# jhamrick/bayesian-quadrature

Hardware: AMD Instinct MI355X
Metric: bq_fit_posterior_throughput (higher is better)
Workload: dtype f64; 1 GPU; C2: d=1 N=1024 M=256 Gaussian integrand, w=dx, s=1e-3; curve_workload=C5 shard: 64 x (d=1 N=2048 M=256), w=dx, s=1e-2, on_curve=True, bordered_system=1344

## Files before the change

### bayesian-quadrature_amd/csrc/k_panel.hip

```cpp
#include "host.h"
#include "gram.h"
#include "trsm.h"
#include "slab.h"

namespace bqh {

template <int D>
void launch_assemble_d(bq_ctx *c, const double *pts, long pstride, const double *y, long ystride,
                       const GaussParams *gp, int gpstride, double *A, long lda, long astride,
                       Layout L, int batch, const FirstStep &fs, int jcols)
{
    dim3 grid((L.ntot + 127) / 128, ((jcols > 0 ? jcols : L.ntot) + 63) / 64, batch);
    if (!fs.S0) {
        hipLaunchKernelGGL(assemble_kernel<D>, grid, dim3(256), 0, c->cur, pts, pstride, y, ystride,
                           gp, gpstride, A, lda, astride, L);
        return;
    }
    const bool regs = c->cfg.first_regs != 0;
    if (regs && grid.y < 3)
        grid.y = 3;
    const long wgs = (long)grid.x * grid.y * grid.z;
    const bool w8 = c->cfg.potf2_8w && wgs <= 2L * c->cus;
#define BQ_ASM_FIRST(NW_, REGS_, STAMP_)                                                           \
    hipLaunchKernelGGL((assemble_first_kernel<D, NW_, REGS_, STAMP_>), grid, dim3(64 * NW_), 0,    \
                       c->cur, pts, pstride, y, ystride, gp, gpstride, A, lda, astride, L, fs.S0,  \
                       fs.lds, fs.sstride, fs.dinv, (long)BQ_DINV_STRIDE, fs.info, fs.scal,        \
                       fs.stamps)
    if constexpr (D == 1) {
        if (fs.stamps) {
            if (w8 && regs)
                BQ_ASM_FIRST(8, true, true);
            else if (w8)
                BQ_ASM_FIRST(8, false, true);
            else if (regs)
                BQ_ASM_FIRST(4, true, true);
            else
                BQ_ASM_FIRST(4, false, true);
            return;
        }
    }
    if (w8 && regs)
        BQ_ASM_FIRST(8, true, false);
    else if (w8)
        BQ_ASM_FIRST(8, false, false);
    else if (regs)
        BQ_ASM_FIRST(4, true, false);
    else
        BQ_ASM_FIRST(4, false, false);
#undef BQ_ASM_FIRST
}

int launch_assemble(bq_ctx *c, int d, const double *pts, long pstride, const double *y,
                    long ystride, const GaussParams *gp, int gpstride, double *A, long lda,
                    long astride, Layout L, int batch, const FirstStep &fs, int jcols)
{
    if (jcols < 0 || (jcols & 63) || jcols > L.ntot || (jcols > 0 && fs.S0))
        return fail(c, BQ_ERR_BAD_ARG, "assemble: column limit");
    if (fs.stamps && (!fs.S0 || d != 1))
        return fail(c, BQ_ERR_BAD_ARG, "assemble: the stamped first launch is one-dimensional");
    const double cols = jcols > 0 ? jcols : L.ntot;
    Bracket br(c, BQ_K_GRAM, 8.0 * cols * (L.ntot - 0.5 * cols + 0.5) * batch);
    switch (d) {
    case 1: launch_assemble_d<1>(c, pts, pstride, y, ystride, gp, gpstride, A, lda, astride, L, batch, fs, jcols); break;
    case 2: launch_assemble_d<2>(c, pts, pstride, y, ystride, gp, gpstride, A, lda, astride, L, batch, fs, jcols); break;
    case 3: launch_assemble_d<3>(c, pts, pstride, y, ystride, gp, gpstride, A, lda, astride, L, batch, fs, jcols); break;
    case 4: launch_assemble_d<4>(c, pts, pstride, y, ystride, gp, gpstride, A, lda, astride, L, batch, fs, jcols); break;
    case 5: launch_assemble_d<5>(c, pts, pstride, y, ystride, gp, gpstride, A, lda, astride, L, batch, fs, jcols); break;
    case 6: launch_assemble_d<6>(c, pts, pstride, y, ystride, gp, gpstride, A, lda, astride, L, batch, fs, jcols); break;
    case 7: launch_assemble_d<7>(c, pts, pstride, y, ystride, gp, gpstride, A, lda, astride, L, batch, fs, jcols); break;
    case 8: launch_assemble_d<8>(c, pts, pstride, y, ystride, gp, gpstride, A, lda, astride, L, batch, fs, jcols); break;
    default: return fail(c, BQ_ERR_BAD_ARG, "d must be in 1..%d", BQ_MAXD);
    }
    HIPCHK(c, hipGetLastError());
    return BQ_OK;
}

int launch_assemble_region(bq_ctx *c, const GramSeed &sd, double *A, long lda, long astride, int m,
                           int n, int batch)
{
    if (m <= 0 || n <= 0)
        return BQ_OK;
    if ((m & 63) || (n & 63) || (sd.r & 63) || (sd.c & 63))
        return fail(c, BQ_ERR_BAD_ARG, "assemble_region: multiples of 64");
    Bracket br(c, BQ_K_GRAM, 8.0 * m * n * batch);
    const dim3 grid((m + 127) / 128, n / 64, batch);
#define BQ_ASM_REGION(D_)                                                                          \
    case D_:                                                                                       \
        hipLaunchKernelGGL(assemble_region_kernel<D_>, grid, dim3(256), 0, c->cur, sd.pts,         \
                           sd.pstride, sd.y, sd.ystride, sd.gp, sd.gpstride, A, lda, astride, sd.L, \
                           sd.r, sd.c, m, n);                                                      \
        break;
    switch (sd.d) {
        BQ_ASM_REGION(1)
        BQ_ASM_REGION(2)
        BQ_ASM_REGION(3)
        BQ_ASM_REGION(4)
        BQ_ASM_REGION(5)
        BQ_ASM_REGION(6)
        BQ_ASM_REGION(7)
        BQ_ASM_REGION(8)
    default:
        return fail(c, BQ_ERR_BAD_ARG, "d must be in 1..%d", BQ_MAXD);
    }
#undef BQ_ASM_REGION
    HIPCHK(c, hipGetLastError());
    return BQ_OK;
}

int launch_potf2(bq_ctx *c, double *A, long lda, long astride, int j0, double *dinv, long dstride,
                 int *info, int batch)
{
    Bracket br(c, BQ_K_POTF2, 64.0 * 64 * 64 / 3.0 * batch);
    if (c->cfg.potf2_8w && batch <= c->cus)
        hipLaunchKernelGGL(potf2_kernel<8>, dim3(1, 1, batch), dim3(512), 0, c->cur, A, lda, astride,
                           j0, dinv, dstride, info);
    else
        hipLaunchKernelGGL(potf2_kernel<4>, dim3(1, 1, batch), dim3(256), 0, c->cur, A, lda, astride,
                           j0, dinv, dstride, info);
    HIPCHK(c, hipGetLastError());
    return BQ_OK;
}

int launch_potrf_wg(bq_ctx *c, double *A, long lda, long astride, int kb, double *rec, long rstride,
                    int *info, int col0, int batch)
{
    Bracket br(c, BQ_K_POTF2, (double)kb * kb * kb / 3.0 * batch);
    hipLaunchKernelGGL(potrf_wg_kernel, dim3(batch), dim3(512), 0, c->cur, A, lda, astride, kb, rec,
                       rstride, info, col0);
    HIPCHK(c, hipGetLastError());
    return BQ_OK;
}

int launch_trsm_blk(bq_ctx *c, double *X, long ldx, long xstride, int m, const double *L11,
                    long ldl, long lstride, const double *dinv, long dstride, int batch)
{
    if (m <= 0)
        return BQ_OK;
    Bracket br(c, BQ_K_TRSM, 64.0 * 64 * (double)m * batch);
    hipLaunchKernelGGL(trsm_blk_kernel, dim3((m + 63) / 64, 1, batch), dim3(256), 0, c->cur, X, ldx,
                       xstride, m, L11, ldl, lstride, dinv, dstride);
    HIPCHK(c, hipGetLastError());
    return BQ_OK;
}

int launch_diag_winv(bq_ctx *c, const double *L, long ldl, int npad, double *dw)
{
    hipLaunchKernelGGL(diag_winv_kernel, dim3(npad / 64), dim3(256), 0, c->stream, L, ldl, dw);
    HIPCHK(c, hipGetLastError());
    return BQ_OK;
}

int launch_panel_step(bq_ctx *c, double *A, long lda, long astride, int batch, int nrb,
                      double *Sin, double *Sout, long lds, long sstride, int K0, int j0,
                      double *dinv_in, double *dinv_out, int has_next, int first, double *SL,
                      int *info, double work)
{
    Bracket br(c, BQ_K_GEMM, work);
    const bool beside_bulk = c->sharing != 0 && (long)nrb * batch > 64;
    if (c->cfg.potf2_8w && !beside_bulk && (long)nrb * batch <= c->cus)
        hipLaunchKernelGGL(panel_step_kernel<8>, dim3(nrb, 1, batch), dim3(512), 0, c->cur, A, lda,
                           astride, Sin, Sout, lds, sstride, K0, j0, dinv_in, dinv_out,
                           (long)BQ_DINV_STRIDE, has_next, first, SL, info);
    else
        hipLaunchKernelGGL(panel_step_kernel<4>, dim3(nrb, 1, batch), dim3(256), 0, c->cur, A, lda,
                           astride, Sin, Sout, lds, sstride, K0, j0, dinv_in, dinv_out,
                           (long)BQ_DINV_STRIDE, has_next, first, SL, info);
    HIPCHK(c, hipGetLastError());
    return BQ_OK;
}

int launch_slab_first(bq_ctx *c, double *A, long lda, long astride, int batch, double *S, long lds,
                      long sstride, int ntot, double *dinv, int *info, int col0, long dstride)
{
    Bracket br(c, BQ_K_POTF2, 64.0 * 64 * 64 / 3.0 * batch);
    hipLaunchKernelGGL(slab_first_kernel, dim3(ntot / 64, 1, batch), dim3(256), 0, c->cur, A, lda,
                       astride, S, lds, sstride, ntot, dinv, dstride, info, col0);
    HIPCHK(c, hipGetLastError());
    return BQ_OK;
}

static long slab8_limit(const bq_ctx *c)
{
    return (long)(c->cfg.slab8_rounds > 1 ? c->cfg.slab8_rounds : 1) * c->cus;
}

int launch_slab_step(bq_ctx *c, double *A, long lda, long astride, int batch, double *Sin,
                     double *Sout, long lds, long sstride, int ntot, int j0, double *dinv_in,
                     double *dinv_out, int fnext, int last, int *info, int col0,
                     const SlabOut &out, long long *stamps, double work, long dstride)
{
    const int T = (ntot - j0 - 64) / 64;
    Bracket br(c, BQ_K_SYRK_SMALL, work);
    const long wgs = (long)T * (T + 1) / 2 * batch;
    const bool w8 = c->cfg.potf2_8w && wgs <= slab8_limit(c);
    if (stamps && w8)
        hipLaunchKernelGGL((slab_step_kernel<true, 8>), dim3(T * (T + 1) / 2, 1, batch), dim3(512), 0,
                           c->cur, A, lda, astride, Sin, Sout, lds, sstride, ntot, j0, dinv_in,
                           dinv_out, dstride, fnext, last, info, col0, stamps, out);
    else if (stamps)
        hipLaunchKernelGGL((slab_step_kernel<true, 4>), dim3(T * (T + 1) / 2, 1, batch), dim3(256), 0,
                           c->cur, A, lda, astride, Sin, Sout, lds, sstride, ntot, j0, dinv_in,
                           dinv_out, dstride, fnext, last, info, col0, stamps, out);
    else if (w8)
        hipLaunchKernelGGL((slab_step_kernel<false, 8>), dim3(T * (T + 1) / 2, 1, batch), dim3(512),
                           0, c->cur, A, lda, astride, Sin, Sout, lds, sstride, ntot, j0, dinv_in,
                           dinv_out, dstride, fnext, last, info, col0,
                           (long long *)nullptr, out);
    else
        hipLaunchKernelGGL((slab_step_kernel<false, 4>), dim3(T * (T + 1) / 2, 1, batch), dim3(256),
                           0, c->cur, A, lda, astride, Sin, Sout, lds, sstride, ntot, j0, dinv_in,
                           dinv_out, dstride, fnext, last, info, col0,
                           (long long *)nullptr, out);
    HIPCHK(c, hipGetLastError());
    return BQ_OK;
}

}
```

### bayesian-quadrature_amd/csrc/launch_config.h

```cpp
#pragma once
#include <hip/hip_runtime.h>

#pragma GCC visibility push(default)
#include "../../include/bqhip.h"
#pragma GCC visibility pop

#include <cstdio>
#include <cstdlib>

#define BQ_LAUNCH_SWITCHES(X)                                                                       \
    X(lookahead, "BQ_LOOKAHEAD", 1)                                                                 \
                 \
    X(la_min, "BQ_LA_MIN", 3072)                                                                    \
                                 \
    X(diag_first, "BQ_DIAG_FIRST", 1)                                                               \
              \
    X(df_sweep, "BQ_DF_SWEEP", 1)                                                                   \
                                               \
    X(df_wg, "BQ_DF_WG", -1)                                                                        \
                                             \
    X(df_wg_rows, "BQ_DF_WG_ROWS", 1000)                                                            \
                       \
    X(df_early, "BQ_DF_EARLY", 1)                                                                   \
                                                  \
    X(trsv_flow, "BQ_TRSV_FLOW", 1)                                                                 \
                                                                                      \
    X(pair_border, "BQ_PAIR_BORDER", 1)                                                             \
            \
    X(solve_kcopy, "BQ_SOLVE_KCOPY", 1)                                                             \
                                              \
    X(gemm_lds, "BQ_GEMM_LDS", 1)                                                                   \
                             \
    X(fold_readout, "BQ_FOLD_READOUT", 1)                                                           \
                                                                           \
    X(asm_fuse, "BQ_ASM_FUSE", 1)                                                                   \
                                                                            \
    X(potf2_8w, "BQ_POTF2_8W", 1)                                                                   \
                           \
    X(first_regs, "BQ_FIRST_REGS", 1)                                                               \
                              \
    X(slab8_rounds, "BQ_SLAB8_ROUNDS", 1 << 20)                                                     \
                        \
    X(gemm_ksplit, "BQ_GEMM_KSPLIT", 1)                                                             \
                  \
    X(gemm_tile, "BQ_GEMM_TILE", 0)                                                                 \
                                                                                     \
    X(use_graph, "BQ_GRAPH", 1)                                                                     \
               \
    X(nb_override, nullptr, 0)

struct LaunchConfig {
#define X(member, env, def) int member = def;
    BQ_LAUNCH_SWITCHES(X)
#undef X
    static LaunchConfig from_env()
    {
        LaunchConfig cfg;
        static const struct {
            const char *env;
            int LaunchConfig::*member;
        } switches[] = {
#define X(member, env, def) {env, &LaunchConfig::member},
            BQ_LAUNCH_SWITCHES(X)
#undef X
        };
        for (const auto &sw : switches)
            if (const char *e = sw.env ? std::getenv(sw.env) : nullptr)
                cfg.*sw.member = std::atoi(e);
        return cfg;
    }
    friend bool operator==(const LaunchConfig &a, const LaunchConfig &b)
    {
#define X(member, env, def) if (a.member != b.member) return false;
        BQ_LAUNCH_SWITCHES(X)
#undef X
        return true;
    }
    friend bool operator!=(const LaunchConfig &a, const LaunchConfig &b) { return !(a == b); }
};

struct CaptureStats {
    long captures = 0;
    long replays = 0;
    long drops = 0;
};

struct CapturedSeq {
    hipGraph_t graph = nullptr;
    hipGraphExec_t exec = nullptr;
    enum State { NotTried, Ready, Unavailable } state = NotTried;
    LaunchConfig cfg;
    CapturedSeq() = default;
    CapturedSeq(const CapturedSeq &) = delete;
    CapturedSeq &operator=(const CapturedSeq &) = delete;
    ~CapturedSeq() { drop(); }
    void drop()
    {
        if (exec)
            (void)hipGraphExecDestroy(exec);
        if (graph)
            (void)hipGraphDestroy(graph);
        exec = nullptr;
        graph = nullptr;
        state = NotTried;
    }
    template <class Ctx, class F>
    int run(Ctx *c, F &&enqueue)
    {
        if (!c->cfg.use_graph || c->prof || !c->own_stream || c->cur != c->stream)
            return enqueue();
        if (state == Ready && cfg != c->cfg) {
            drop();
            ++c->graphs.drops;
        }
        if (state == NotTried) {
            state = Unavailable;
            cfg = c->cfg;
            if (hipStreamBeginCapture(c->stream, hipStreamCaptureModeRelaxed) == hipSuccess) {
                const int st = enqueue();
                const hipError_t e = hipStreamEndCapture(c->stream, &graph);
                if (st == BQ_OK && e == hipSuccess && graph &&
                    hipGraphInstantiate(&exec, graph, nullptr, nullptr, 0) == hipSuccess) {
                    state = Ready;
                    ++c->graphs.captures;
                }
            }
            if (state != Ready) {
                exec = nullptr;
                drop();
                state = Unavailable;
                (void)hipGetLastError();
            }
        }
        if (state != Ready)
            return enqueue();
        const hipError_t e = hipGraphLaunch(exec, c->stream);
        if (e != hipSuccess) {
            std::snprintf(c->err, sizeof c->err, "hipGraphLaunch failed: %s", hipGetErrorString(e));
            return BQ_ERR_HIP;
        }
        ++c->graphs.replays;
        return BQ_OK;
    }
};
```

### bayesian-quadrature_amd/csrc/slab.h

```cpp
#pragma once
#include "common.h"
#include "potf2.h"


__device__ __forceinline__ void slab_load16(const double *__restrict__ S, long lds,
                                            double (&t)[4][4])
{
#pragma unroll
    for (int c = 0; c < 4; ++c)
#pragma unroll
        for (int r = 0; r < 4; ++r)
            t[c][r] = S[(long)(16 * c + 4 * r) * lds];
}

__device__ __forceinline__ void slab_solve16(const double (&t)[4][4], const double (&la)[4][3][4],
                                             const double (&wneg)[4][4], double4_t (&x)[4])
{
#pragma unroll
    for (int c = 0; c < 4; ++c) {
        double4_t acc = {-t[c][0], -t[c][1], -t[c][2], -t[c][3]};
#pragma unroll
        for (int bb = 0; bb < c; ++bb)
#pragma unroll
            for (int r = 0; r < 4; ++r)
                acc = __builtin_amdgcn_mfma_f64_16x16x4f64(la[c][bb][r], x[bb][r], acc, 0, 0, 0);
        double4_t xc = {0.0, 0.0, 0.0, 0.0};
#pragma unroll
        for (int r = 0; r < 4; ++r)
            xc = __builtin_amdgcn_mfma_f64_16x16x4f64(wneg[c][r], acc[r], xc, 0, 0, 0);
        x[c] = xc;
    }
}

__device__ __forceinline__ void slab_frags(const double *Fs, int l15, int l4, double (&la)[4][3][4],
                                           double (&wneg)[4][4])
{
    const double *Ws = Fs + 6 * 256;
#pragma unroll
    for (int c = 0; c < 4; ++c)
#pragma unroll
        for (int r = 0; r < 4; ++r)
            wneg[c][r] = Ws[256 * c + 64 * r + l15 + 16 * l4];
#pragma unroll
    for (int c = 1; c < 4; ++c)
#pragma unroll
        for (int bb = 0; bb < c; ++bb)
#pragma unroll
            for (int r = 0; r < 4; ++r)
                la[c][bb][r] = Fs[256 * ((c * (c - 1)) / 2 + bb) + l15 + 16 * (l4 + 4 * r)];
}

#define BQ_SLAB_FW (10 * 256)
#define DIAG_NB(w) ((w) < 2 ? 3 : 2)
#define DIAG_RB(w, s) ((w) == 0 ? ((s) > 0 ? 1 : 0) : ((w) == 1 ? 2 : 3))
#define DIAG_CB(w, s) ((w) == 0 ? ((s) == 2 ? 1 : 0) : (((w) == 3 ? 2 : 0) + ((w) >= 2 && (s) == 2 ? 1 : (s))))

__device__ __forceinline__ void slab_load_blocks8(Potf2FT<8> &st, const double *Bs, int w, int lane)
{
    const int rb = lane >> 4, i = lane & 15;
#pragma unroll
    for (int q = 0; q < 2; ++q)
#pragma unroll
        for (int s = 0; s < 4; ++s) {
            const int c = 4 * (8 * q + w) + s;
            const int cb = c >> 4, rc = rb > cb ? rb : cb;
            const double v = Bs[256 * ((rc * (rc + 1)) / 2 + cb) + i + 16 * (c & 15)];
            st.a[q][s] = rb >= cb ? v : 0.0;
        }
}

__device__ __forceinline__ void slab_corner_factor8(double *Ab, long lda, int j0, double *dinv_b,
                                                    int *info_b, double *plds, long long *stamps,
                                                    double *logdet)
{
    const int lane = threadIdx.x & 63;
    const int w = __builtin_amdgcn_readfirstlane(threadIdx.x >> 6);
    if (stamps && threadIdx.x == 0)
        stamps[0] = (long long)__builtin_amdgcn_s_memtime();
    Potf2FT<8> st;
    slab_load_blocks8(st, plds + 4096, w, lane);
    potf2f_run<8>(st, Ab, lda, j0, dinv_b, info_b, plds, stamps, logdet);
}

template <bool STAMP, int NW = 4>
__global__ __launch_bounds__(64 * NW, NW == 4 ? 2 : 1) void slab_step_kernel(double *__restrict__ A, long lda,
                                                        long astride,
                                                        const double *__restrict__ Sin,
                                                        double *__restrict__ Sout, long lds,
                                                        long sstride, int ntot, int j0,
                                                        const double *__restrict__ din,
                                                        double *__restrict__ dout, long dstride,
                                                        int factor_next, int last,
                                                        int *__restrict__ info, int col0,
                                                        long long *stamps, SlabOut out)
{
#define BQ_SSTAMP(k, dep)                                                                          \
    if (STAMP) {                                                                                   \
        asm volatile("" ::"v"(dep));                                                               \
        __builtin_amdgcn_sched_barrier(0);                                                         \
        if (blockIdx.x == 0 && blockIdx.z == 0 && threadIdx.x == 0)                                \
            stamps[k] = (long long)__builtin_amdgcn_s_memtime();                                   \
        __builtin_amdgcn_sched_barrier(0);                                                         \
    }
    BQ_SSTAMP(0, 0)
    __shared__ __attribute__((aligned(16))) double plds[4096 + BQ_SLAB_FW];
    double *const Qs = plds;
    double *const Ts = plds;
    __builtin_amdgcn_s_setprio(3);
    const int b = blockIdx.z;
    const int lane = threadIdx.x & 63;
    const int wave = __builtin_amdgcn_readfirstlane(threadIdx.x >> 6);
    int bx, by;
    tri_decode(blockIdx.x, bx, by);
    A += (long)b * astride;
    Sin += (long)b * sstride;
    Sout += (long)b * sstride;
    din += (long)b * dstride;
    dout += (long)b * dstride;
    const int r0 = j0 + 64;
    const int Rb = r0 + 64 * bx, Cb = r0 + 64 * by;
    const int l15 = lane & 15, l4 = lane >> 4;
    if (NW == 8 && wave >= 4) {
        if (bx != by) {
            const int wq = wave - 4;
            double tq[4][4];
            slab_load16(Sin + Cb + 16 * wq + l15 + (long)l4 * lds, lds, tq);
            __syncthreads();
            double la[4][3][4], wneg[4][4];
            slab_frags(plds + 4096, l15, l4, la, wneg);
            double4_t xq[4];
            slab_solve16(tq, la, wneg, xq);
#pragma unroll
            for (int c = 0; c < 4; ++c)
#pragma unroll
                for (int r = 0; r < 4; ++r)
                    Qs[(16 * c + l4 + 4 * r) * 64 + 16 * wq + l15] = xq[c][r];
            __syncthreads();
            return;
        }
        __syncthreads();
        __syncthreads();
        if (blockIdx.x == 0 && factor_next) {
            __syncthreads();
            slab_corner_factor8(A + r0 + (long)r0 * lda, lda, col0 + r0, dout, info + b, plds,
                                nullptr, out.scal ? out.scal + 4 * b + 1 : nullptr);
        }
        return;
    }

    double la[4][3][4], wneg[4][4], tp[4][4], tq[4][4];
    double4_t acc[4];
    {
        double *Fs = plds + 4096;
        double *Ws = plds + 4096 + 6 * 256;
        {
            const int t = threadIdx.x, ti = t & 15, tk = t >> 4;
            const double *L11 = A + j0 + (long)j0 * lda + ti + (long)tk * lda;
            double f[6], wv[4];
#pragma unroll
            for (int c = 1; c < 4; ++c)
#pragma unroll
                for (int bb = 0; bb < c; ++bb)
                    f[(c * (c - 1)) / 2 + bb] = L11[16 * c + (long)(16 * bb) * lda];
#pragma unroll
            for (int q = 0; q < 4; ++q)
                wv[q] = din[64 + 256 * q + t];
            if (NW == 4)
                slab_load16(Sin + Cb + 16 * wave + l15 + (long)l4 * lds, lds, tq);
            slab_load16(Sin + Rb + 16 * wave + l15 + (long)l4 * lds, lds, tp);
            {
                const bool dg = bx == by;
#pragma unroll
                for (int cb = 0; cb < 4; ++cb) {
                    const int sb = cb < 2 ? cb : 2;
                    const int ro = dg ? 16 * DIAG_RB(wave, sb) : 16 * wave;
                    const int co = dg ? 16 * DIAG_CB(wave, sb) : 16 * cb;
                    const double *Cin = A + Rb + ro + l15 + (long)(Cb + co + l4) * lda;
#pragma unroll
                    for (int r = 0; r < 4; ++r)
                        acc[cb][r] = Cin[(long)(4 * r) * lda];
                }
            }
            __builtin_amdgcn_sched_barrier(0);
#pragma unroll
            for (int q = 0; q < 6; ++q)
                Fs[256 * q + t] = f[q];
#pragma unroll
            for (int q = 0; q < 4; ++q)
                Ws[256 * q + t] = -wv[q];
        }
        __syncthreads();
        slab_frags(Fs, l15, l4, la, wneg);
    }
    BQ_SSTAMP(1, la[3][2][3] + wneg[3][3])
    double4_t xp[4];
    if (NW == 4 && bx != by) {
        double4_t xq[4];
        slab_solve16(tq, la, wneg, xq);
#pragma unroll
        for (int c = 0; c < 4; ++c)
#pragma unroll
            for (int r = 0; r < 4; ++r)
                Qs[(16 * c + l4 + 4 * r) * 64 + 16 * wave + l15] = xq[c][r];
    }
    slab_solve16(tp, la, wneg, xp);
    if (bx == by) {
#pragma unroll
        for (int c = 0; c < 4; ++c)
#pragma unroll
            for (int r = 0; r < 4; ++r)
                Qs[(16 * c + l4 + 4 * r) * 64 + 16 * wave + l15] = xp[c][r];
    }
    BQ_SSTAMP(2, xp[3][3])
    __builtin_amdgcn_sched_barrier(0);
#pragma unroll
    for (int cb = 0; cb < 4; ++cb)
        if (cb < 3 || bx != by) {
#pragma unroll
            for (int r = 0; r < 4; ++r) {
                double v = -acc[cb][r];
                asm volatile("" : "+v"(v));
                acc[cb][r] = v;
            }
        }
    __builtin_amdgcn_sched_barrier(0);
    if (by == 0) {
        double *Lw = A + Rb + 16 * wave + l15 + (long)(j0 + l4) * lda;
#pragma unroll
        for (int c = 0; c < 4; ++c)
#pragma unroll
            for (int r = 0; r < 4; ++r)
                Lw[(long)(16 * c + 4 * r) * lda] = xp[c][r];
    }
    __syncthreads();
    BQ_SSTAMP(3, acc[1][3] + acc[0][0])
    if (bx == by) {
        const int rb0 = DIAG_RB(wave, 0), rb1 = DIAG_RB(wave, 1), rb2 = DIAG_RB(wave, 2);
        const int cb0 = DIAG_CB(wave, 0), cb1 = DIAG_CB(wave, 1), cb2 = DIAG_CB(wave, 2);
#pragma unroll
        for (int c = 0; c < 4; ++c)
#pragma unroll
            for (int r = 0; r < 4; ++r) {
                const double *qrow = Qs + (16 * c + l4 + 4 * r) * 64 + l15;
                acc[0] = __builtin_amdgcn_mfma_f64_16x16x4f64(qrow[16 * cb0], qrow[16 * rb0], acc[0],
                                                              0, 0, 0);
                acc[1] = __builtin_amdgcn_mfma_f64_16x16x4f64(qrow[16 * cb1], qrow[16 * rb1], acc[1],
                                                              0, 0, 0);
                acc[2] = __builtin_amdgcn_mfma_f64_16x16x4f64(qrow[16 * cb2], qrow[16 * rb2],
                                                              acc[2], 0, 0, 0);
            }
    } else {
#pragma unroll
        for (int c = 0; c < 4; ++c)
#pragma unroll
            for (int r = 0; r < 4; ++r) {
                const double pf = xp[c][r];
                const double *qrow = Qs + (16 * c + l4 + 4 * r) * 64 + l15;
#pragma unroll
                for (int cb = 0; cb < 4; ++cb)
                    acc[cb] =
                        __builtin_amdgcn_mfma_f64_16x16x4f64(qrow[16 * cb], pf, acc[cb], 0, 0, 0);
            }
    }
    BQ_SSTAMP(4, acc[1][3] + acc[0][0])
    if (blockIdx.x == 0 && factor_next) {
        if constexpr (NW == 8) {
            double *Bs = plds + 4096;
#pragma unroll
            for (int sb = 0; sb < 3; ++sb)
                if (sb < DIAG_NB(wave)) {
                    const int rb = DIAG_RB(wave, sb), cb = DIAG_CB(wave, sb);
#pragma unroll
                    for (int r = 0; r < 4; ++r)
                        Bs[256 * ((rb * (rb + 1)) / 2 + cb) + l15 + 16 * (l4 + 4 * r)] = -acc[sb][r];
                }
            __syncthreads();
            slab_corner_factor8(A + r0 + (long)r0 * lda, lda, col0 + r0, dout, info + b, plds,
                                (STAMP && blockIdx.z == 0) ? stamps + 5 : nullptr,
                                out.scal ? out.scal + 4 * b + 1 : nullptr);
            return;
        }
        __syncthreads();
#pragma unroll
        for (int sb = 0; sb < 3; ++sb)
            if (sb < DIAG_NB(wave)) {
#pragma unroll
                for (int r = 0; r < 4; ++r)
                    Ts[16 * DIAG_RB(wave, sb) + l15 +
                       64 * (16 * DIAG_CB(wave, sb) + l4 + 4 * r)] = -acc[sb][r];
            }
        __syncthreads();
        potf2_body<NW>(A + r0 + (long)r0 * lda, lda, col0 + r0, dout, info + b, plds, Ts, 64,
                       (STAMP && blockIdx.z == 0) ? stamps + 5 : nullptr,
                       out.scal ? out.scal + 4 * b + 1 : nullptr);
        return;
    }
    const bool to_s = by == 0 && bx > 0 && !last;
    double *Cout = to_s ? Sout + Rb + 16 * wave + l15 + (long)l4 * lds
                        : A + Rb + 16 * wave + l15 + (long)(Cb + l4) * lda;
    const long ldo = to_s ? lds : lda;
#define BQ_SLAB_EMIT(ROW_, COL_, S_)                                                               \
    {                                                                                              \
        const int row_ = (ROW_), col_ = (COL_);                                                    \
        const double s_ = (S_);                                                                    \
        if (row_ == col_ && row_ >= out.npad && row_ < out.npad + out.M && out.var)                \
            out.var[(long)b * out.mstride + (row_ - out.npad)] = s_;                               \
        if (row_ == out.yrow) {                                                                    \
            if (col_ >= out.npad && col_ < out.npad + out.M && out.mean)                           \
                out.mean[(long)b * out.mstride + (col_ - out.npad)] = -s_;                         \
            if (col_ == out.yrow) {                                                                \
                const double qf_ = -s_, ld_ = out.scal[4 * b + 1];                                 \
                out.scal[4 * b + 2] = qf_;                                                         \
                out.scal[4 * b + 0] =                                                              \
                    -0.5 * qf_ - 0.5 * ld_ - 0.5 * (double)out.n * 1.8378770664093453;             \
            }                                                                                      \
        }                                                                                          \
    }
    const bool emit = last && out.scal != nullptr;
    if (bx == by) {
#pragma unroll
        for (int sb = 0; sb < 3; ++sb)
            if (sb < DIAG_NB(wave)) {
                double *Cd = A + Rb + 16 * DIAG_RB(wave, sb) + l15 +
                             (long)(Cb + 16 * DIAG_CB(wave, sb) + l4) * lda;
#pragma unroll
                for (int r = 0; r < 4; ++r)
                    Cd[(long)(4 * r) * lda] = -acc[sb][r];
                if (emit) {
#pragma unroll
                    for (int r = 0; r < 4; ++r)
                        BQ_SLAB_EMIT(Rb + 16 * DIAG_RB(wave, sb) + l15,
                                     Cb + 16 * DIAG_CB(wave, sb) + l4 + 4 * r, -acc[sb][r])
                }
            }
    } else {
#pragma unroll
        for (int cb = 0; cb < 4; ++cb)
#pragma unroll
            for (int r = 0; r < 4; ++r)
                Cout[(long)(16 * cb + 4 * r) * ldo] = -acc[cb][r];
        if (emit) {
#pragma unroll
            for (int cb = 0; cb < 4; ++cb)
#pragma unroll
                for (int r = 0; r < 4; ++r)
                    BQ_SLAB_EMIT(Rb + 16 * wave + l15, Cb + 16 * cb + l4 + 4 * r, -acc[cb][r])
        }
    }
#undef BQ_SLAB_EMIT
#undef BQ_SSTAMP
}


template <int D, int NW>
__device__ __forceinline__ void first_block_regs(Potf2FT<NW> &st, const double *__restrict__ pts,
                                                 const GaussParams &gm, double *__restrict__ A,
                                                 long lda, const Layout &L, int wv, int lane)
{
    constexpr int NG = 16 / NW;
    constexpr int GQ = 4 * NG * D <= 32 ? NG : 1;
    Layout L0 = L;
    L0.yrow = -1;
    GaussParams g;
    g.c = gm.c, g.s2 = gm.s2;
#pragma unroll
    for (int k = 0; k < D; ++k)
        g.nh[k] = gm.nh[k];
    const bool pi = lane < L.n;
    double xi[D];
#pragma unroll
    for (int k = 0; k < D; ++k)
        xi[k] = pts[k + (long)(pi ? lane : 0) * D];
#pragma unroll
    for (int q0 = 0; q0 < NG; q0 += GQ) {
        double xj[GQ][4][D];
#pragma unroll
        for (int q = 0; q < GQ; ++q)
#pragma unroll
            for (int s = 0; s < 4; ++s) {
                const int c = 4 * (NW * (q0 + q) + wv) + s;
#pragma unroll
                for (int k = 0; k < D; ++k)
                    xj[q][s][k] = pts[k + (long)(c < L.n ? c : 0) * D];
            }
        __builtin_amdgcn_sched_barrier(0);
#pragma unroll
        for (int q = 0; q < GQ; ++q)
#pragma unroll
            for (int s = 0; s < 4; ++s) {
                const int c = 4 * (NW * (q0 + q) + wv) + s;
                st.a[q0 + q][s] =
                    bordered_entry_flat<D>(lane, c, pi, c < L.n, xi, xj[q][s], g, L0, 0.0);
            }
    }
#pragma unroll
    for (int q = 0; q < NG; ++q)
#pragma unroll
        for (int s = 0; s < 4; ++s)
            PIN(st.a[q][s]);
#pragma unroll
    for (int q = 0; q < NG; ++q)
#pragma unroll
        for (int s = 0; s < 4; ++s) {
            const int c = 4 * (NW * q + wv) + s;
            if (lane < c)
                A[lane + (long)c * lda] = st.a[q][s];
        }
}

template <int D, int NW = 4, bool REGS = true, bool STAMP = false>
__global__ __launch_bounds__(64 * NW) void assemble_first_kernel(
    const double *__restrict__ pts, long pstride, const double *__restrict__ y, long ystride,
    const GaussParams *__restrict__ gp, int gpstride, double *__restrict__ A, long lda,
    long astride, Layout L, double *__restrict__ S0, long lds, long sstride,
    double *__restrict__ dinv, long dstride, int *__restrict__ info, double *__restrict__ scal,
    long long *stamps)
{
    __shared__ __attribute__((aligned(16))) double plds[BQ_POTF2_LDS_DOUBLES];
    const int b = blockIdx.z;
    const bool corner = blockIdx.x == 0 && blockIdx.y == 0;
    long long *const st0 = (STAMP && corner && b == 0) ? stamps : nullptr;
    if (st0 && threadIdx.x == 0)
        st0[0] = (long long)__builtin_amdgcn_s_memtime();
    A += (long)b * astride;
    if constexpr (REGS) {
        if (blockIdx.x == 0 && blockIdx.y == 2) {
            if (NW == 4 || threadIdx.x < 256)
                assemble_tile<D>(pts + (long)b * pstride, y + (long)b * ystride,
                                 gp[(long)b * gpstride], A, lda, L, S0 + (long)b * sstride, lds, 64,
                                 0, 128);
            return;
        }
        if (corner) {
            __builtin_amdgcn_s_setprio(3);
            const int lane = threadIdx.x & 63;
            Potf2FT<NW> st;
            first_block_regs<D, NW>(st, pts + (long)b * pstride, gp[(long)b * gpstride], A, lda, L,
                                    (int)(threadIdx.x >> 6), lane);
            if (st0) {
                asm volatile("" ::"v"(st.a[0][0]));
                if (threadIdx.x == 0)
                    st0[1] = st0[2] = (long long)__builtin_amdgcn_s_memtime();
            }
            potf2f_run<NW>(st, A, lda, 0, dinv + (long)b * dstride, info + b, plds,
                           st0 ? st0 + 2 : nullptr, scal ? scal + 4 * b + 1 : nullptr, L.n, true);
            return;
        }
    }
    if (NW == 4 || threadIdx.x < 256)
        assemble_tile<D>(pts + (long)b * pstride, y + (long)b * ystride, gp[(long)b * gpstride],
                         A, lda, L, S0 + (long)b * sstride, lds);
    if (!REGS && corner) {
        if (threadIdx.x == 0) {
            info[b] = 0;
            if (scal)
                scal[4 * b + 1] = 0.0;
        }
        asm volatile("s_waitcnt vmcnt(0)" ::: "memory");
        __syncthreads();
        if (st0 && threadIdx.x == 0)
            st0[1] = (long long)__builtin_amdgcn_s_memtime();
        __builtin_amdgcn_s_setprio(3);
        potf2_body<NW>(A, lda, 0, dinv + (long)b * dstride, info + b, plds, nullptr, 0,
                       st0 ? st0 + 2 : nullptr, scal ? scal + 4 * b + 1 : nullptr, L.n);
    }
}

__global__ __launch_bounds__(256) void slab_first_kernel(double *__restrict__ A, long lda,
                                                         long astride, double *__restrict__ S,
                                                         long lds, long sstride, int ntot,
                                                         double *__restrict__ dinv, long dstride,
                                                         int *__restrict__ info, int col0)
{
    __shared__ __attribute__((aligned(16))) double plds[BQ_POTF2_LDS_DOUBLES];
    const int b = blockIdx.z;
    A += (long)b * astride;
    if (blockIdx.x == 0) {
        __builtin_amdgcn_s_setprio(3);
        potf2_body(A, lda, col0, dinv + (long)b * dstride, info + b, plds);
        return;
    }
    const int i = 64 * (int)blockIdx.x + (threadIdx.x & 63);
    const int jb = (threadIdx.x >> 6) * 16;
    if (i < ntot) {
        double *dst = S + (long)b * sstride + i + (long)jb * lds;
        const double *src = A + i + (long)jb * lda;
#pragma unroll
        for (int j = 0; j < 16; ++j)
            dst[(long)j * lds] = src[(long)j * lda];
    }
}

template <int NW = 4>
__global__ __launch_bounds__(64 * NW) void panel_step_kernel(double *__restrict__ A, long lda,
                                                         long astride,
                                                         const double *__restrict__ Sin,
                                                         double *__restrict__ Sout, long lds,
                                                         long sstride, int K0, int j0,
                                                         const double *__restrict__ din,
                                                         double *__restrict__ dout, long dstride,
                                                         int has_next, int first,
                                                         double *__restrict__ SL,
                                                         int *__restrict__ info)
{
    __shared__ __attribute__((aligned(16))) double plds[BQ_POTF2_LDS_DOUBLES];
    double *const Qs = plds;
    double *const Ts = plds;
    __builtin_amdgcn_s_setprio(3);
    const int b = blockIdx.z;
    const int lane = threadIdx.x & 63;
    const int wave = __builtin_amdgcn_readfirstlane(threadIdx.x >> 6);
    A += (long)b * astride;
    Sin += (long)b * sstride;
    Sout += (long)b * sstride;
    din += (long)b * dstride;
    dout += (long)b * dstride;
    const int r0 = j0 + 64;
    const int Rb = r0 + 64 * blockIdx.x;
    const int l15 = lane & 15, l4 = lane >> 4;
    SL += (long)b * 4096;
    const double *Sp = first ? A + (long)j0 * lda : Sin;
    const long ldsp = first ? lda : lds;
    if (!first && j0 - K0 == 64 && blockIdx.x == 0) {
        double *dst = A + j0 + (long)(j0 - 64) * lda;
        for (int e = threadIdx.x; e < 4096; e += 64 * NW)
            dst[(e & 63) + (long)(e >> 6) * lda] = SL[e];
    }
    if (NW == 8 && wave >= 4 && (!has_next || blockIdx.x == 0)) {
        if (!has_next)
            return;
        __syncthreads();
        __syncthreads();
        __syncthreads();
        potf2_body<8>(A + r0 + (long)r0 * lda, lda, r0, dout, info + b, plds, Ts, 64);
        return;
    }

    double la[4][3][4], wneg[4][4];
    {
        const double *L11 = A + j0 + (long)j0 * lda + l15 + (long)l4 * lda;
        const double *W = din + 64 + l15 + 16 * l4;
#pragma unroll
        for (int c = 0; c < 4; ++c)
#pragma unroll
            for (int r = 0; r < 4; ++r)
                wneg[c][r] = -W[256 * c + 64 * r];
#pragma unroll
        for (int c = 1; c < 4; ++c)
#pragma unroll
            for (int bb = 0; bb < c; ++bb)
#pragma unroll
                for (int r = 0; r < 4; ++r)
                    la[c][bb][r] = L11[16 * c + (long)(16 * bb + 4 * r) * lda];
    }
    double4_t xp[4];
    if (has_next && blockIdx.x != 0 && (NW == 4 || wave >= 4)) {
        const int wq = wave & 3;
        double4_t xq[4];
        double tq[4][4];
        slab_load16(Sp + r0 + 16 * wq + l15 + (long)l4 * ldsp, ldsp, tq);
        slab_solve16(tq, la, wneg, xq);
#pragma unroll
        for (int c = 0; c < 4; ++c)
#pragma unroll
            for (int r = 0; r < 4; ++r)
                Qs[(16 * c + l4 + 4 * r) * 64 + 16 * wq + l15] = xq[c][r];
        if (NW == 8) {
            __syncthreads();
            return;
        }
    }
    {
        double tp[4][4];
        slab_load16(Sp + Rb + 16 * wave + l15 + (long)l4 * ldsp, ldsp, tp);
        slab_solve16(tp, la, wneg, xp);
    }
    {
        const bool side = first && has_next && blockIdx.x == 0 && gridDim.x > 1;
        double *Lw = side ? SL + 16 * wave + l15 + 64 * l4
                          : A + Rb + 16 * wave + l15 + (long)(j0 + l4) * lda;
        const long ldw = side ? 64 : lda;
#pragma unroll
        for (int c = 0; c < 4; ++c)
#pragma unroll
            for (int r = 0; r < 4; ++r)
                Lw[(long)(16 * c + 4 * r) * ldw] = xp[c][r];
    }
    if (!has_next)
        return;
    if (blockIdx.x == 0) {
#pragma unroll
        for (int c = 0; c < 4; ++c)
#pragma unroll
            for (int r = 0; r < 4; ++r)
                Qs[(16 * c + l4 + 4 * r) * 64 + 16 * wave + l15] = xp[c][r];
    }
    const double *Cin = A + Rb + 16 * wave + l15 + (long)(r0 + l4) * lda;
    double4_t acc[4];
#pragma unroll
    for (int cb = 0; cb < 4; ++cb)
#pragma unroll
        for (int r = 0; r < 4; ++r)
            acc[cb][r] = -Cin[(long)(16 * cb + 4 * r) * lda];
    {
        const double *Pg = A + Rb + 16 * wave + l15 + (long)(K0 + l4) * lda;
        const double *Qg = A + r0 + l15 + (long)(K0 + l4) * lda;
        const int kend = j0 - K0;
        double pa[4], qa[4][4], pb[4], qb[4][4];
#define BQ_PANEL_LOAD(PF, QF, KK)                                                                  \
    _Pragma("unroll") for (int t = 0; t < 4; ++t)                                                  \
    {                                                                                              \
        PF[t] = Pg[(long)((KK) + 4 * t) * lda];                                                    \
        _Pragma("unroll") for (int cb = 0; cb < 4; ++cb) QF[t][cb] =                               \
            Qg[16 * cb + (long)((KK) + 4 * t) * lda];                                              \
    }
#define BQ_PANEL_MFMA(PF, QF)                                                                      \
    _Pragma("unroll") for (int t = 0; t < 4; ++t) _Pragma("unroll") for (int cb = 0; cb < 4; ++cb) \
        acc[cb] = __builtin_amdgcn_mfma_f64_16x16x4f64(QF[t][cb], PF[t], acc[cb], 0, 0, 0);
        if (kend > 0) {
            BQ_PANEL_LOAD(pa, qa, 0)
            for (int kk = 0; kk < kend; kk += 32) {
                BQ_PANEL_LOAD(pb, qb, kk + 16)
                __builtin_amdgcn_sched_barrier(0);
                BQ_PANEL_MFMA(pa, qa)
                __builtin_amdgcn_sched_barrier(0);
                const int kn = kk + 32 < kend ? kk + 32 : kk;
                BQ_PANEL_LOAD(pa, qa, kn)
                __builtin_amdgcn_sched_barrier(0);
                BQ_PANEL_MFMA(pb, qb)
                __builtin_amdgcn_sched_barrier(0);
            }
        }
#undef BQ_PANEL_LOAD
#undef BQ_PANEL_MFMA
    }
    __syncthreads();
#pragma unroll
    for (int c = 0; c < 4; ++c)
#pragma unroll
        for (int r = 0; r < 4; ++r) {
            const double pf = xp[c][r];
            const double *qrow = Qs + (16 * c + l4 + 4 * r) * 64 + l15;
#pragma unroll
            for (int cb = 0; cb < 4; ++cb)
                acc[cb] = __builtin_amdgcn_mfma_f64_16x16x4f64(qrow[16 * cb], pf, acc[cb], 0, 0, 0);
        }
    if (blockIdx.x == 0) {
        __syncthreads();
#pragma unroll
        for (int cb = 0; cb < 4; ++cb)
#pragma unroll
            for (int r = 0; r < 4; ++r)
                Ts[16 * wave + l15 + 64 * (16 * cb + l4 + 4 * r)] = -acc[cb][r];
        __syncthreads();
        potf2_body<NW>(A + r0 + (long)r0 * lda, lda, r0, dout, info + b, plds, Ts, 64);
        return;
    }
    double *Cout = Sout + Rb + 16 * wave + l15 + (long)l4 * lds;
#pragma unroll
    for (int cb = 0; cb < 4; ++cb)
#pragma unroll
        for (int r = 0; r < 4; ++r)
            Cout[(long)(16 * cb + 4 * r) * lds] = -acc[cb][r];
}

__device__ __forceinline__ void wg_update32(double *__restrict__ C, long ldc,
                                            const double *__restrict__ P,
                                            const double *__restrict__ Q, long ldp, int row0,
                                            int col0, int lane)
{
    const int l15 = lane & 15, l4 = lane >> 4;
    double pa[16][2], qa[16][2], cold[2][2][4];
#pragma unroll
    for (int h = 0; h < 2; ++h) {
        const double *pp = P + row0 + 16 * h + l15 + (long)l4 * ldp;
        const double *qq = Q + col0 + 16 * h + l15 + (long)l4 * ldp;
#pragma unroll
        for (int ks = 0; ks < 16; ++ks) {
            pa[ks][h] = pp[(long)(4 * ks) * ldp];
            qa[ks][h] = qq[(long)(4 * ks) * ldp];
        }
    }
#pragma unroll
    for (int tm = 0; tm < 2; ++tm)
#pragma unroll
        for (int tn = 0; tn < 2; ++tn)
#pragma unroll
            for (int rr = 0; rr < 4; ++rr)
                cold[tm][tn][rr] =
                    C[(row0 + 16 * tm + l15) + (long)(col0 + 16 * tn + l4 + 4 * rr) * ldc];
    __builtin_amdgcn_sched_barrier(0);
    double4_t acc[2][2];
#pragma unroll
    for (int tm = 0; tm < 2; ++tm)
#pragma unroll
        for (int tn = 0; tn < 2; ++tn)
            acc[tm][tn] = (double4_t){0.0, 0.0, 0.0, 0.0};
#pragma unroll
    for (int ks = 0; ks < 16; ++ks)
#pragma unroll
        for (int tm = 0; tm < 2; ++tm)
#pragma unroll
            for (int tn = 0; tn < 2; ++tn)
                acc[tm][tn] =
                    __builtin_amdgcn_mfma_f64_16x16x4f64(qa[ks][tn], pa[ks][tm], acc[tm][tn], 0, 0, 0);
#pragma unroll
    for (int tm = 0; tm < 2; ++tm)
#pragma unroll
        for (int tn = 0; tn < 2; ++tn) {
            if (col0 + 16 * tn >= row0 + 16 * tm + 16)
                continue;
#pragma unroll
            for (int rr = 0; rr < 4; ++rr)
                C[(row0 + 16 * tm + l15) + (long)(col0 + 16 * tn + l4 + 4 * rr) * ldc] =
                    cold[tm][tn][rr] - acc[tm][tn][rr];
        }
}

__global__ __launch_bounds__(512) void potrf_wg_kernel(double *__restrict__ A, long lda,
                                                       long astride, int kb,
                                                       double *__restrict__ rec, long rstride,
                                                       int *__restrict__ info, int col0)
{
    __shared__ __attribute__((aligned(16))) double plds[BQ_POTF2_LDS_DOUBLES];
    __builtin_amdgcn_s_setprio(3);
    const int b = blockIdx.x;
    A += (long)b * astride;
    rec += (long)b * rstride;
    const int lane = threadIdx.x & 63;
    const int wave = __builtin_amdgcn_readfirstlane(threadIdx.x >> 6);
    const int l15 = lane & 15, l4 = lane >> 4;
    const int ns = kb >> 6;
    for (int s = 0; s < ns; ++s) {
        double *Ass = A + 64 * s + (long)(64 * s) * lda;
        double *rs = rec + (long)s * BQ_DINV_HALF;
        potf2_body<8>(Ass, lda, col0 + 64 * s, rs, info + b, plds);
        asm volatile("s_waitcnt vmcnt(0)" ::: "memory");
        __syncthreads();
        const int nr = ns - s - 1;
        if (nr == 0)
            break;
        const int r0 = 64 * (s + 1);
        {
            double la[4][3][4], wneg[4][4];
            const double *L11 = Ass + l15 + (long)l4 * lda;
            const double *W = rs + 64 + l15 + 16 * l4;
#pragma unroll
            for (int c = 0; c < 4; ++c)
#pragma unroll
                for (int r = 0; r < 4; ++r)
                    wneg[c][r] = -W[256 * c + 64 * r];
#pragma unroll
            for (int c = 1; c < 4; ++c)
#pragma unroll
                for (int bb = 0; bb < c; ++bb)
#pragma unroll
                    for (int r = 0; r < 4; ++r)
                        la[c][bb][r] = L11[16 * c + (long)(16 * bb + 4 * r) * lda];
            for (int task = wave; task < 4 * nr; task += 8) {
                double *Xr = A + r0 + 16 * task + l15 + (long)(64 * s + l4) * lda;
                double t[4][4];
                double4_t x[4];
                slab_load16(Xr, lda, t);
                slab_solve16(t, la, wneg, x);
#pragma unroll
                for (int c = 0; c < 4; ++c)
#pragma unroll
                    for (int r = 0; r < 4; ++r)
                        Xr[(long)(16 * c + 4 * r) * lda] = x[c][r];
            }
        }
        asm volatile("s_waitcnt vmcnt(0)" ::: "memory");
        __syncthreads();
        {
            const double *Pn = A + r0 + (long)(64 * s) * lda;
            double *Cn = A + r0 + (long)r0 * lda;
            const int ntask = 4 * (nr * (nr + 1) / 2);
            for (int task = wave; task < ntask; task += 8) {
                int ti, tj;
                tri_decode(task >> 2, ti, tj);
                const int q = task & 3;
                const int row0 = 64 * ti + 32 * (q & 1), cl0 = 64 * tj + 32 * (q >> 1);
                if (cl0 > row0)
                    continue;
                wg_update32(Cn, lda, Pn, Pn, lda, row0, cl0, lane);
            }
        }
        asm volatile("s_waitcnt vmcnt(0)" ::: "memory");
        __syncthreads();
    }
}
```

Baseline: 4269 problems/s.

## Pipeline diagonal slab-step tiles across waves with per-column TRSM/SYRK overlap

Adds a PIPE variant of the 8-wave slab step kernel, on by default through BQ_DIAG_PIPE. For diagonal tiles, waves 0-3 compute the triangular-solve panel one 16-column chunk at a time and publish each chunk to LDS. Waves 4-7 apply the SYRK update for that chunk right after each barrier instead of waiting for the whole panel. The intent is to overlap the dependent TRSM chain with the diagonal rank update and so shorten the critical path of each step. The cost is more barriers, more code paths, and register pressure in the 8-wave kernel.

```diff
diff --git a/bayesian-quadrature_amd/csrc/k_panel.hip b/bayesian-quadrature_amd/csrc/k_panel.hip
--- a/bayesian-quadrature_amd/csrc/k_panel.hip
+++ b/bayesian-quadrature_amd/csrc/k_panel.hip
@@ -193,26 +193,27 @@
     Bracket br(c, BQ_K_SYRK_SMALL, work);
     const long wgs = (long)T * (T + 1) / 2 * batch;
     const bool w8 = c->cfg.potf2_8w && wgs <= slab8_limit(c);
-    if (stamps && w8)
-        hipLaunchKernelGGL((slab_step_kernel<true, 8>), dim3(T * (T + 1) / 2, 1, batch), dim3(512), 0,
-                           c->cur, A, lda, astride, Sin, Sout, lds, sstride, ntot, j0, dinv_in,
-                           dinv_out, dstride, fnext, last, info, col0, stamps, out);
+    const bool pipe = w8 && c->cfg.diag_pipe != 0;
+#define BQ_SLAB_STEP(STAMP_, NW_, PIPE_)                                                           \
+    hipLaunchKernelGGL((slab_step_kernel<STAMP_, NW_, PIPE_>), dim3(T * (T + 1) / 2, 1, batch),    \
+                       dim3(64 * NW_), 0, c->cur, A, lda, astride, Sin, Sout, lds, sstride, ntot,  \
+                       j0, dinv_in, dinv_out, dstride, fnext, last, info, col0,                    \
+                       STAMP_ ? stamps : (long long *)nullptr, out)
+    if (stamps && pipe)
+        BQ_SLAB_STEP(true, 8, true);
+    else if (stamps && w8)
+        BQ_SLAB_STEP(true, 8, false);
     else if (stamps)
-        hipLaunchKernelGGL((slab_step_kernel<true, 4>), dim3(T * (T + 1) / 2, 1, batch), dim3(256), 0,
-                           c->cur, A, lda, astride, Sin, Sout, lds, sstride, ntot, j0, dinv_in,
-                           dinv_out, dstride, fnext, last, info, col0, stamps, out);
+        BQ_SLAB_STEP(true, 4, false);
+    else if (pipe)
+        BQ_SLAB_STEP(false, 8, true);
     else if (w8)
-        hipLaunchKernelGGL((slab_step_kernel<false, 8>), dim3(T * (T + 1) / 2, 1, batch), dim3(512),
-                           0, c->cur, A, lda, astride, Sin, Sout, lds, sstride, ntot, j0, dinv_in,
-                           dinv_out, dstride, fnext, last, info, col0,
-                           (long long *)nullptr, out);
-    else
-        hipLaunchKernelGGL((slab_step_kernel<false, 4>), dim3(T * (T + 1) / 2, 1, batch), dim3(256),
-                           0, c->cur, A, lda, astride, Sin, Sout, lds, sstride, ntot, j0, dinv_in,
-                           dinv_out, dstride, fnext, last, info, col0,
-                           (long long *)nullptr, out);
-    HIPCHK(c, hipGetLastError());
-    return BQ_OK;
-}
-
-}
+        BQ_SLAB_STEP(false, 8, false);
+    else
+        BQ_SLAB_STEP(false, 4, false);
+#undef BQ_SLAB_STEP
+    HIPCHK(c, hipGetLastError());
+    return BQ_OK;
+}
+
+}
diff --git a/bayesian-quadrature_amd/csrc/launch_config.h b/bayesian-quadrature_amd/csrc/launch_config.h
--- a/bayesian-quadrature_amd/csrc/launch_config.h
+++ b/bayesian-quadrature_amd/csrc/launch_config.h
@@ -40,6 +40,8 @@
     X(first_regs, "BQ_FIRST_REGS", 1)                                                               \
                               \
     X(slab8_rounds, "BQ_SLAB8_ROUNDS", 1 << 20)                                                     \
+                       \
+    X(diag_pipe, "BQ_DIAG_PIPE", 1)                                                                 \
                         \
     X(gemm_ksplit, "BQ_GEMM_KSPLIT", 1)                                                             \
                   \
diff --git a/bayesian-quadrature_amd/csrc/slab.h b/bayesian-quadrature_amd/csrc/slab.h
--- a/bayesian-quadrature_amd/csrc/slab.h
+++ b/bayesian-quadrature_amd/csrc/slab.h
@@ -82,7 +82,7 @@
     potf2f_run<8>(st, Ab, lda, j0, dinv_b, info_b, plds, stamps, logdet);
 }
 
-template <bool STAMP, int NW = 4>
+template <bool STAMP, int NW = 4, bool PIPE = false>
 __global__ __launch_bounds__(64 * NW, NW == 4 ? 2 : 1) void slab_step_kernel(double *__restrict__ A, long lda,
                                                         long astride,
                                                         const double *__restrict__ Sin,
@@ -101,6 +101,31 @@
         if (blockIdx.x == 0 && blockIdx.z == 0 && threadIdx.x == 0)                                \
             stamps[k] = (long long)__builtin_amdgcn_s_memtime();                                   \
         __builtin_amdgcn_sched_barrier(0);                                                         \
+    }
+#define BQ_SSTAMP_T(k, dep, tid)                                                                   \
+    if (STAMP) {                                                                                   \
+        asm volatile("" ::"v"(dep));                                                               \
+        __builtin_amdgcn_sched_barrier(0);                                                         \
+        if (blockIdx.x == 0 && blockIdx.z == 0 && threadIdx.x == (tid))                            \
+            stamps[k] = (long long)__builtin_amdgcn_s_memtime();                                   \
+        __builtin_amdgcn_sched_barrier(0);                                                         \
+    }
+#define BQ_SLAB_EMIT(ROW_, COL_, S_)                                                               \
+    {                                                                                              \
+        const int row_ = (ROW_), col_ = (COL_);                                                    \
+        const double s_ = (S_);                                                                    \
+        if (row_ == col_ && row_ >= out.npad && row_ < out.npad + out.M && out.var)                \
+            out.var[(long)b * out.mstride + (row_ - out.npad)] = s_;                               \
+        if (row_ == out.yrow) {                                                                    \
+            if (col_ >= out.npad && col_ < out.npad + out.M && out.mean)                           \
+                out.mean[(long)b * out.mstride + (col_ - out.npad)] = -s_;                         \
+            if (col_ == out.yrow) {                                                                \
+                const double qf_ = -s_, ld_ = out.scal[4 * b + 1];                                 \
+                out.scal[4 * b + 2] = qf_;                                                         \
+                out.scal[4 * b + 0] =                                                              \
+                    -0.5 * qf_ - 0.5 * ld_ - 0.5 * (double)out.n * 1.8378770664093453;             \
+            }                                                                                      \
+        }                                                                                          \
     }
     BQ_SSTAMP(0, 0)
     __shared__ __attribute__((aligned(16))) double plds[4096 + BQ_SLAB_FW];
@@ -120,6 +145,174 @@
     const int r0 = j0 + 64;
     const int Rb = r0 + 64 * bx, Cb = r0 + 64 * by;
     const int l15 = lane & 15, l4 = lane >> 4;
+    if constexpr (NW == 8 && PIPE) {
+        if (bx == by) {
+            if (wave >= 4) {
+                const int wu = wave - 4;
+                const int rb0 = DIAG_RB(wu, 0), rb1 = DIAG_RB(wu, 1), rb2 = DIAG_RB(wu, 2);
+                const int cb0 = DIAG_CB(wu, 0), cb1 = DIAG_CB(wu, 1), cb2 = DIAG_CB(wu, 2);
+                double4_t acc[3];
+    #pragma unroll
+                for (int sb = 0; sb < 3; ++sb) {
+                    const double *Cin = A + Rb + 16 * DIAG_RB(wu, sb) + l15 +
+                                        (long)(Cb + 16 * DIAG_CB(wu, sb) + l4) * lda;
+    #pragma unroll
+                    for (int r = 0; r < 4; ++r)
+                        acc[sb][r] = Cin[(long)(4 * r) * lda];
+                }
+                __syncthreads();
+                __builtin_amdgcn_sched_barrier(0);
+    #pragma unroll
+                for (int sb = 0; sb < 3; ++sb)
+    #pragma unroll
+                    for (int r = 0; r < 4; ++r) {
+                        double v = -acc[sb][r];
+                        asm volatile("" : "+v"(v));
+                        acc[sb][r] = v;
+                    }
+                __builtin_amdgcn_sched_barrier(0);
+    #pragma unroll
+                for (int c = 0; c < 4; ++c) {
+                    if (c > 0)
+                        BQ_SSTAMP_T(15 + c, acc[0][0], 256)
+                    __builtin_amdgcn_sched_barrier(0);
+                    __syncthreads();
+                    __builtin_amdgcn_sched_barrier(0);
+                    double qa[4][3], qb[4][3];
+    #pragma unroll
+                    for (int r = 0; r < 4; ++r) {
+                        const double *qrow = Qs + (16 * c + l4 + 4 * r) * 64 + l15;
+                        qa[r][0] = qrow[16 * cb0], qb[r][0] = qrow[16 * rb0];
+                        qa[r][1] = qrow[16 * cb1], qb[r][1] = qrow[16 * rb1];
+                        qa[r][2] = qrow[16 * cb2], qb[r][2] = qrow[16 * rb2];
+                    }
+                    __builtin_amdgcn_sched_barrier(0);
+    #pragma unroll
+                    for (int r = 0; r < 4; ++r) {
+                        acc[0] = __builtin_amdgcn_mfma_f64_16x16x4f64(qa[r][0], qb[r][0], acc[0], 0, 0, 0);
+                        acc[1] = __builtin_amdgcn_mfma_f64_16x16x4f64(qa[r][1], qb[r][1], acc[1], 0, 0, 0);
+                        acc[2] = __builtin_amdgcn_mfma_f64_16x16x4f64(qa[r][2], qb[r][2], acc[2], 0, 0, 0);
+                    }
+                }
+                BQ_SSTAMP_T(4, acc[1][3] + acc[0][0], 256)
+                if (blockIdx.x == 0 && factor_next) {
+                    double *Bs = plds + 4096;
+    #pragma unroll
+                    for (int sb = 0; sb < 3; ++sb)
+                        if (sb < DIAG_NB(wu)) {
+                            const int rb = DIAG_RB(wu, sb), cb = DIAG_CB(wu, sb);
+    #pragma unroll
+                            for (int r = 0; r < 4; ++r)
+                                Bs[256 * ((rb * (rb + 1)) / 2 + cb) + l15 + 16 * (l4 + 4 * r)] = -acc[sb][r];
+                        }
+                    __syncthreads();
+                    slab_corner_factor8(A + r0 + (long)r0 * lda, lda, col0 + r0, dout, info + b, plds,
+                                        nullptr, out.scal ? out.scal + 4 * b + 1 : nullptr);
+                    return;
+                }
+                const bool emit = last && out.scal != nullptr;
+    #pragma unroll
+                for (int sb = 0; sb < 3; ++sb)
+                    if (sb < DIAG_NB(wu)) {
+                        double *Cd = A + Rb + 16 * DIAG_RB(wu, sb) + l15 +
+                                     (long)(Cb + 16 * DIAG_CB(wu, sb) + l4) * lda;
+    #pragma unroll
+                        for (int r = 0; r < 4; ++r)
+                            Cd[(long)(4 * r) * lda] = -acc[sb][r];
+                        if (emit) {
+    #pragma unroll
+                            for (int r = 0; r < 4; ++r)
+                                BQ_SLAB_EMIT(Rb + 16 * DIAG_RB(wu, sb) + l15,
+                                             Cb + 16 * DIAG_CB(wu, sb) + l4 + 4 * r, -acc[sb][r])
+                        }
+                    }
+                return;
+            }
+            double la[4][3][4], wneg[4][4], tp[4][4];
+            double *Fs = plds + 4096;
+            {
+                double *Ws = plds + 4096 + 6 * 256;
+                const int t = threadIdx.x, ti = t & 15, tk = t >> 4;
+                const double *L11 = A + j0 + (long)j0 * lda + ti + (long)tk * lda;
+                double f[6], wv[4];
+#pragma unroll
+                for (int c = 1; c < 4; ++c)
+#pragma unroll
+                    for (int bb = 0; bb < c; ++bb)
+                        f[(c * (c - 1)) / 2 + bb] = L11[16 * c + (long)(16 * bb) * lda];
+#pragma unroll
+                for (int q = 0; q < 4; ++q)
+                    wv[q] = din[64 + 256 * q + t];
+                slab_load16(Sin + Rb + 16 * wave + l15 + (long)l4 * lds, lds, tp);
+                __builtin_amdgcn_sched_barrier(0);
+#pragma unroll
+                for (int q = 0; q < 6; ++q)
+                    Fs[256 * q + t] = f[q];
+#pragma unroll
+                for (int q = 0; q < 4; ++q)
+                    Ws[256 * q + t] = -wv[q];
+            }
+            __syncthreads();
+            {
+                const double *Ws = Fs + 6 * 256;
+                double4_t x[4];
+#define BQ_PIPE_FRAGS(C_)                                                                          \
+    do {                                                                                           \
+        _Pragma("unroll") for (int r = 0; r < 4; ++r) wneg[C_][r] =                                \
+            Ws[256 * (C_) + 64 * r + l15 + 16 * l4];                                               \
+        _Pragma("unroll") for (int bb = 0; bb < (C_); ++bb) _Pragma("unroll") for (int r = 0;      \
+                                                                                   r < 4; ++r)     \
+            la[C_][bb][r] = Fs[256 * (((C_) * ((C_) - 1)) / 2 + bb) + l15 + 16 * (l4 + 4 * r)];    \
+    } while (0)
+                BQ_PIPE_FRAGS(0);
+                BQ_PIPE_FRAGS(1);
+                BQ_SSTAMP(1, wneg[0][3] + wneg[1][3])
+#pragma unroll
+                for (int c = 0; c < 4; ++c) {
+                    double4_t a = {-tp[c][0], -tp[c][1], -tp[c][2], -tp[c][3]};
+#pragma unroll
+                    for (int bb = 0; bb < c; ++bb)
+#pragma unroll
+                        for (int r = 0; r < 4; ++r)
+                            a = __builtin_amdgcn_mfma_f64_16x16x4f64(la[c][bb][r], x[bb][r], a, 0, 0, 0);
+                    double4_t xc = {0.0, 0.0, 0.0, 0.0};
+#pragma unroll
+                    for (int r = 0; r < 4; ++r)
+                        xc = __builtin_amdgcn_mfma_f64_16x16x4f64(wneg[c][r], a[r], xc, 0, 0, 0);
+                    x[c] = xc;
+#pragma unroll
+                    for (int r = 0; r < 4; ++r)
+                        Qs[(16 * c + l4 + 4 * r) * 64 + 16 * wave + l15] = xc[r];
+                    if (c == 0) {
+                        BQ_PIPE_FRAGS(2);
+                    }
+                    if (c == 1) {
+                        BQ_PIPE_FRAGS(3);
+                    }
+                    if (c > 0)
+                        BQ_SSTAMP(18 + c, xc[3])
+                    __syncthreads();
+                }
+#undef BQ_PIPE_FRAGS
+                BQ_SSTAMP(2, x[3][3])
+                if (by == 0) {
+                    double *Lw = A + Rb + 16 * wave + l15 + (long)(j0 + l4) * lda;
+#pragma unroll
+                    for (int c = 0; c < 4; ++c)
+#pragma unroll
+                        for (int r = 0; r < 4; ++r)
+                            Lw[(long)(16 * c + 4 * r) * lda] = x[c][r];
+                }
+                if (blockIdx.x == 0 && factor_next) {
+                    __syncthreads();
+                    slab_corner_factor8(A + r0 + (long)r0 * lda, lda, col0 + r0, dout, info + b,
+                                        plds, (STAMP && blockIdx.z == 0) ? stamps + 5 : nullptr,
+                                        out.scal ? out.scal + 4 * b + 1 : nullptr);
+                }
+                return;
+            }
+        }
+    }
     if (NW == 8 && wave >= 4) {
         if (bx != by) {
             const int wq = wave - 4;
@@ -263,7 +456,7 @@
             }
     }
     BQ_SSTAMP(4, acc[1][3] + acc[0][0])
-    if (blockIdx.x == 0 && factor_next) {
+    if (!(NW == 8 && PIPE) && blockIdx.x == 0 && factor_next) {
         if constexpr (NW == 8) {
             double *Bs = plds + 4096;
 #pragma unroll
@@ -299,23 +492,6 @@
     double *Cout = to_s ? Sout + Rb + 16 * wave + l15 + (long)l4 * lds
                         : A + Rb + 16 * wave + l15 + (long)(Cb + l4) * lda;
     const long ldo = to_s ? lds : lda;
-#define BQ_SLAB_EMIT(ROW_, COL_, S_)                                                               \
-    {                                                                                              \
-        const int row_ = (ROW_), col_ = (COL_);                                                    \
-        const double s_ = (S_);                                                                    \
-        if (row_ == col_ && row_ >= out.npad && row_ < out.npad + out.M && out.var)                \
-            out.var[(long)b * out.mstride + (row_ - out.npad)] = s_;                               \
-        if (row_ == out.yrow) {                                                                    \
-            if (col_ >= out.npad && col_ < out.npad + out.M && out.mean)                           \
-                out.mean[(long)b * out.mstride + (col_ - out.npad)] = -s_;                         \
-            if (col_ == out.yrow) {                                                                \
-                const double qf_ = -s_, ld_ = out.scal[4 * b + 1];                                 \
-                out.scal[4 * b + 2] = qf_;                                                         \
-                out.scal[4 * b + 0] =                                                              \
-                    -0.5 * qf_ - 0.5 * ld_ - 0.5 * (double)out.n * 1.8378770664093453;             \
-            }                                                                                      \
-        }                                                                                          \
-    }
     const bool emit = last && out.scal != nullptr;
     if (bx == by) {
 #pragma unroll
@@ -348,6 +524,7 @@
         }
     }
 #undef BQ_SLAB_EMIT
+#undef BQ_SSTAMP_T
 #undef BQ_SSTAMP
 }
 
```

Measured after the change: 4519 problems/s (median of 6 runs). +5.9%, better.
